# leospeidel/Colate

Hardware: AMD Instinct MI355X
Metric: bootstrap replicates/sec to EM convergence, whole-genome SGDP mut, 20 epochs (higher is better)
Workload: dtype f64

## Files before the change

### colate_amd/csrc/em_kernel_impl.hpp

```cpp
#pragma once
#include <hip/hip_runtime.h>

#include <cstdlib>
#include <cstring>
#include <type_traits>

#include "em_kernels.h"
#include "em_math.hpp"

namespace {

constexpr int kWave = 64;
enum { O_W = 0, O_N, O_D, kNumBinArrays };
enum { G_LAM = 0, G_INV, G_XA, G_P, G_BETA, G_CS, G_S, G_PW, kNumGather };
constexpr int G_Q = kNumGather;
constexpr int num_gather_rows(int nch, bool tput) { return (nch >= 2 || !tput) ? kNumGather + 1 : kNumGather; }
constexpr int tail_scratch_arrays(int nch, bool tput) { return nch >= 2 ? (tput ? 3 : 6) : 0; }

__device__ __forceinline__ double readlane_d(double v, int lane) {
  int lo = __builtin_amdgcn_readlane(__double2loint(v), lane);
  int hi = __builtin_amdgcn_readlane(__double2hiint(v), lane);
  return __hiloint2double(hi, lo);
}

template <int CTRL, int ROW_MASK = 0xf, bool BOUND = false>
__device__ __forceinline__ double dpp_d(double old, double v) {
  int lo = __builtin_amdgcn_update_dpp(__double2loint(old), __double2loint(v), CTRL, ROW_MASK, 0xf, BOUND);
  int hi = __builtin_amdgcn_update_dpp(__double2hiint(old), __double2hiint(v), CTRL, ROW_MASK, 0xf, BOUND);
  return __hiloint2double(hi, lo);
}
constexpr int ROW_SHR1 = 0x111, ROW_SHR2 = 0x112, ROW_SHR4 = 0x114, ROW_SHR8 = 0x118;
constexpr int ROW_SHL1 = 0x101, ROW_SHL2 = 0x102, ROW_SHL4 = 0x104, ROW_SHL8 = 0x108;
constexpr int ROW_BCAST15 = 0x142, ROW_BCAST31 = 0x143, WAVE_SHR1 = 0x138, WAVE_SHL1 = 0x130;


__device__ __forceinline__ double wave_prefix_sum(double v, int rows = 4) {
  v += dpp_d<ROW_SHR1, 0xf, true>(0.0, v);
  v += dpp_d<ROW_SHR2, 0xf, true>(0.0, v);
  v += dpp_d<ROW_SHR4, 0xf, true>(0.0, v);
  v += dpp_d<ROW_SHR8, 0xf, true>(0.0, v);
  if (rows > 1) v += dpp_d<ROW_BCAST15, 0xa>(0.0, v);
  if (rows > 2) v += dpp_d<ROW_BCAST31, 0xc>(0.0, v);
  return v;
}
__device__ __forceinline__ double wave_suffix_sum(double v, int lane, int rows = 4) {
  v += dpp_d<ROW_SHL1, 0xf, true>(0.0, v);
  v += dpp_d<ROW_SHL2, 0xf, true>(0.0, v);
  v += dpp_d<ROW_SHL4, 0xf, true>(0.0, v);
  v += dpp_d<ROW_SHL8, 0xf, true>(0.0, v);
  if (rows > 1) {
    const double r1 = readlane_d(v, 16);
    double add = 0.0;
    if (rows > 2) {
      const double r2 = readlane_d(v, 32), r3 = readlane_d(v, 48);
      const double s23 = r2 + r3, s123 = r1 + s23;
      const int row = lane >> 4;
      add = row == 0 ? s123 : (row == 1 ? s23 : (row == 2 ? r3 : 0.0));
    } else {
      add = (lane >> 4) == 0 ? r1 : 0.0;
    }
    v = v + add;
  }
  return v;
}
__device__ __forceinline__ void wave_affine_scan(double& a, double& b, int rows = 4, const double* nosrc = nullptr) {
#define COLATE_AFF_STEP(CTRL, RM, BND, K)                                                                   \
  {                                                                                                         \
    const double as = nosrc ? dpp_d<CTRL, RM, true>(0.0, a) + nosrc[K] : dpp_d<CTRL, RM>(1.0, a);           \
    const double bs = dpp_d<CTRL, RM, BND>(0.0, b);                                                         \
    b = em::fma_(a, bs, b);                                                                                 \
    a = a * as;                                                                                             \
  }
  COLATE_AFF_STEP(ROW_SHR1, 0xf, true, 0)
  COLATE_AFF_STEP(ROW_SHR2, 0xf, true, 1)
  COLATE_AFF_STEP(ROW_SHR4, 0xf, true, 2)
  COLATE_AFF_STEP(ROW_SHR8, 0xf, true, 3)
#undef COLATE_AFF_STEP
  if (rows == 2) {
    const double bs = dpp_d<ROW_BCAST15, 0xa>(0.0, b);
    b = em::fma_(a, bs, b);
  }
#define COLATE_AFF_STEP2(CTRL, RM)                 \
  {                                                \
    const double as = dpp_d<CTRL, RM>(1.0, a);     \
    const double bs = dpp_d<CTRL, RM>(0.0, b);     \
    b = em::fma_(a, bs, b);                        \
    a = a * as;                                    \
  }
  if (rows > 2) COLATE_AFF_STEP2(ROW_BCAST15, 0xa)
  if (rows > 2) COLATE_AFF_STEP2(ROW_BCAST31, 0xc)
#undef COLATE_AFF_STEP2
}

__device__ __forceinline__ double wave_suffix_max(double v, int lane) {
  v = __builtin_fmax(v, dpp_d<ROW_SHL1, 0xf, true>(0.0, v));
  v = __builtin_fmax(v, dpp_d<ROW_SHL2, 0xf, true>(0.0, v));
  v = __builtin_fmax(v, dpp_d<ROW_SHL4, 0xf, true>(0.0, v));
  v = __builtin_fmax(v, dpp_d<ROW_SHL8, 0xf, true>(0.0, v));
  const double r1 = readlane_d(v, 16), r2 = readlane_d(v, 32), r3 = readlane_d(v, 48);
  const double m23 = __builtin_fmax(r2, r3), m123 = __builtin_fmax(r1, m23);
  const int row = lane >> 4;
  return __builtin_fmax(v, row == 0 ? m123 : (row == 1 ? m23 : (row == 2 ? r3 : 0.0)));
}
__device__ __forceinline__ double half_ulp_pos(double z) {
  const int ex = (__double2hiint(z) >> 20) & 0x7ff;
  return ex > 53 ? __hiloint2double((ex - 53) << 20, 0) : 0.0;
}

__device__ __forceinline__ double tail_hneg(double z, double& q) {
  const float a = __builtin_fminf(__builtin_fabsf((float)z), 30.0f);
  const float t = __builtin_amdgcn_rcpf(__builtin_fmaf(0.2316419f, a, 1.0f));
  float poly = __builtin_fmaf(t, 1.330274429f, -1.821255978f);
  poly = __builtin_fmaf(t, poly, 1.781477937f);
  poly = __builtin_fmaf(t, poly, -0.356563782f);
  poly = __builtin_fmaf(t, poly, 0.319381530f);
  poly = poly * t;
  const float phi = 0.3989422804f * __builtin_amdgcn_exp2f(-0.72134752f * (a * a));
  const float qa = phi * poly;
  const float base = __builtin_fmaxf(__builtin_fmaf(-a, qa, phi), 0.0f);
  q = z < 0.0 ? (double)(1.0f - qa) : (double)qa;
  return (z < 0.0 ? -z : 0.0) + (double)base;
}

#ifdef COLATE_EM_STAMPS
__device__ __forceinline__ unsigned long long stamp() {
  unsigned long long t;
  __builtin_amdgcn_sched_barrier(0);
  asm volatile("s_memtime %0\n\ts_waitcnt lgkmcnt(0)" : "=s"(t)::"memory");
  __builtin_amdgcn_sched_barrier(0);
  return t;
}
#define COLATE_STAMP(i)                     \
  {                                         \
    const unsigned long long now_ = stamp(); \
    st_acc[i] += now_ - st_prev;            \
    st_prev = now_;                         \
  }
#define COLATE_PSTAMP(i) pro_t[i] = stamp();
#else
#define COLATE_STAMP(i)
#define COLATE_PSTAMP(i)
#endif

#ifdef COLATE_ABL
#define COLATE_ABL_HAS(b) (((COLATE_ABL) >> (b)) & 1)
#else
#define COLATE_ABL_HAS(b) 0
#endif

#define COLATE_COLD() asm volatile("; cold path")
#define COLATE_STR2(x) #x
#define COLATE_STR(x) COLATE_STR2(x)

__device__ __forceinline__ bool finite_pos(double x) { return x > 0.0 && x < __builtin_inf(); }

__device__ __forceinline__ unsigned long long ballot64(bool p) { return __builtin_amdgcn_ballot_w64(p); }

__device__ __forceinline__ void wave_lds_fence() {
  __builtin_amdgcn_fence(__ATOMIC_RELEASE, "wavefront");
  __builtin_amdgcn_wave_barrier();
  __builtin_amdgcn_fence(__ATOMIC_ACQUIRE, "wavefront");
}

struct BinStat {
  double a_b, cnt, tk, tkn, dtk, da, db;
  double f1, f2, f4, f8;
  int kb, pos;
  bool live, last_bin, is_tail;
};
enum { BF_F1 = 1, BF_F2 = 2, BF_F4 = 4, BF_F8 = 8, BF_TAIL = 16, BF_INRANGE = 32, BF_KB_SHIFT = 8 };

constexpr int em_loop_pad(int mode, int nch, int erows, bool tput, int wpe) {
#ifdef COLATE_LOOP_PAD
  return (COLATE_LOOP_PAD) & 7;
#else
  (void)erows, (void)wpe;
  if (mode != 0) return 0;
#ifdef COLATE_EM_ILP_BUILD
  (void)tput;
  return nch == 1 ? (wpe == 2 ? 5 : 6) : 2;
#else
  (void)nch;
  if (!tput) return 6;
  return 4;
#endif
#endif
}

constexpr int em_loop_pad2(int mode, int nch, bool tput) {
#if defined(COLATE_EM_ILP_BUILD) && !defined(COLATE_LOOP_PAD)
  (void)mode, (void)nch, (void)tput;
  return -1;
#else
  (void)mode, (void)nch, (void)tput;
  return -1;
#endif
}

template <int MODE, int NCH, int EROWS, bool TPUT, int WPE = 0>
__global__ __launch_bounds__(TPUT ? 2 * kWave : 2 * COLATE_EM_MAX_A, WPE ? WPE : ((NCH == 1) ? 3 : (NCH == 2 ? 2 : 1))) void em_kernel(ColateEmArgs p) {
  extern __shared__ double lds[];
  const int E = p.E, A = p.A;
  constexpr int EPAD = NCH * kWave;
  const int NBMAX = (A + kWave - 1) / kWave;
  const int AP = NBMAX * kWave;
  const int APZ = AP + 2;
  const int tid = threadIdx.x, lane = tid & 63;
  constexpr int kSlotShift = (NCH == 1) ? 0 : (NCH == 2 ? 1 : (NCH == 4 ? 2 : (NCH == 8 ? 3 : 4)));
  static_assert(NCH == 1 || NCH == 2 || NCH == 4 || NCH == 8 || NCH == 16, "NCH");
  auto ep_of = [&](int c) { return lane * NCH + c; };
  const int wave = __builtin_amdgcn_readfirstlane(tid >> 6);
  const int role = wave & 1;
  const int grp = wave >> 1;
  const int rep = blockIdx.x;

  double* s_t = lds;
  double* s_ep = s_t + EPAD + 1;
  constexpr int kRows = num_gather_rows(NCH, TPUT);
  double* s_out = s_ep + kRows * EPAD;
  double* s_nd = s_out + 2 * kNumBinArrays * APZ;
  double* s_cfail = s_nd + 4 * EPAD;
  double* s_cnt = s_cfail + 2 * APZ;
  double* s_ll = s_cnt + 2 * APZ;
  double* s_exptab = s_ll + 12;
  double* s_age = s_exptab + em::kExpTableDoubles;
  double* s_tscr = s_age + AP;
  int* s_kb = reinterpret_cast<int*>(s_tscr + tail_scratch_arrays(NCH, TPUT) * APZ);
  int* s_fail = s_kb + AP + 1;
  int* s_misc = s_fail + 8;
  int* s_bflags = s_misc + 4;

#ifdef COLATE_EM_TRACE
  unsigned long long trace_t0;
  asm volatile("s_memtime %0\n\ts_waitcnt lgkmcnt(0)" : "=s"(trace_t0)::"memory");
#endif
#ifdef COLATE_EM_STAMPS
  unsigned long long pro_t[10] = {0, 0, 0, 0, 0, 0, 0, 0, 0, 0};
#endif
  COLATE_PSTAMP(0)
  const double* epochs = p.epochs + (size_t)rep * p.epochs_stride;
  for (int i = tid; i < EPAD + 1; i += blockDim.x) s_t[i] = (i < E) ? epochs[i] : 0.0;
  for (int i = tid; i < kRows * EPAD + 2 * kNumBinArrays * APZ + 4 * EPAD + 4 * APZ; i += blockDim.x) s_ep[i] = 0.0;
  if (tid == 0) {
    s_misc[0] = A;
    s_misc[1] = 0;
    s_misc[2] = 0;
    s_misc[3] = 0;
  }
  if (tid < 8) {
    s_ll[tid] = 0.0;
    s_fail[tid] = 0;
  }
  if (tid < em::kExpTableDoubles) s_exptab[tid] = em::kExpTableDevice[tid];
  __syncthreads();
  COLATE_PSTAMP(1)
  for (int t = tid; t < AP; t += blockDim.x) {
    int kb = E;
    bool has_sh = false, has_ns = false;
    if (t < A) {
      const double a = p.age_grid[t];
      const double c1 = p.cnt_sh[(size_t)rep * A + t];
      const double c2 = p.cnt_ns[(size_t)rep * A + t];
      const double csh = (c1 > 0) ? c1 : 0.0;
      const double cns = (c2 > 0) ? c2 : 0.0;
      int first_gt = 0;
      for (int len = E; len > 0;) {
        const int half = len >> 1;
        if (!(a < s_t[first_gt + half])) {
          first_gt += half + 1;
          len -= half + 1;
        } else {
          len = half;
        }
      }
      kb = first_gt - 1;
      if (kb < 0) kb = 0;
      s_cnt[t] = csh;
      s_cnt[APZ + t] = cns;
      s_age[t] = a;
      has_sh = csh > 0;
      has_ns = cns > 0;
    }
    {
      const unsigned long long m_sh = ballot64(has_sh), m_ns = ballot64(has_ns), m_any = m_sh | m_ns;
      if (m_any != 0 && lane == 0) {
        atomicMin(&s_misc[0], t + (int)__builtin_ctzll(m_any));
        atomicMax(&s_misc[1], t + 64 - (int)__builtin_clzll(m_any));
        atomicAdd(&s_misc[3], (int)__builtin_popcountll(m_sh) + (int)__builtin_popcountll(m_ns));
      }
    }
    s_kb[t] = kb;
  }
  if (tid == 0) s_kb[AP] = E + 1;
  __syncthreads();
  COLATE_PSTAMP(2)
  int nzlo = s_misc[0], nzhi = s_misc[1];
  if (nzlo >= nzhi) {
    nzlo = 0;
    nzhi = 0;
  }
  const int NB = (nzhi - nzlo + 63) / 64 > 0 ? (nzhi - nzlo + 63) / 64 : 1;

  double t_e[NCH], tn_e[NCH], dt_e[NCH], lam_e[NCH];
  bool vstat[NCH], ep_on[NCH];
#pragma unroll
  for (int c = 0; c < NCH; c++) {
    const int e = ep_of(c);
    ep_on[c] = e < E;
    t_e[c] = s_t[e];
    tn_e[c] = 0.0;
    dt_e[c] = 0.0;
    vstat[c] = false;
    lam_e[c] = 0.0;
    if (ep_on[c]) {
      if (e < E - 1) {
        tn_e[c] = s_t[e + 1];
        dt_e[c] = tn_e[c] - t_e[c];
        vstat[c] = (tn_e[c] != 0) && (dt_e[c] > 0);
      } else {
        vstat[c] = true;
      }
      lam_e[c] = p.rates_in[(size_t)rep * p.rates_stride + e];
      if (MODE == 0 && wave == 0) p.out_rates[(size_t)rep * E + e] = lam_e[c];
    }
  }
  COLATE_PSTAMP(3)
  if (tid == 0) s_ll[10] = (nzhi > nzlo) ? (double)s_kb[nzhi - 1] : -1.0;
  const int pos = grp * kWave + lane;
  const int bin = nzlo + pos;
  const bool in_range = (grp < NB) && (bin < nzhi);
  double a_b = 0, cnt = 0, tk = 0, tkn = 0, dtk = 0, da = 0, db = 0;
  int kb = E;
  if (in_range) {
    a_b = p.age_grid[bin];
    cnt = s_cnt[role * APZ + bin];
    kb = s_kb[bin];
    tk = s_t[kb];
    if (kb < E - 1) {
      tkn = s_t[kb + 1];
      dtk = tkn - tk;
    }
    da = a_b - tk;
    db = (kb < E - 1) ? tkn - a_b : 0.0;
  }
  const bool live = in_range && cnt > 0;
  const bool last_bin = (kb == E - 1);
  double f1 = 0, f2 = 0, f4 = 0, f8 = 0;
  bool is_tail = false;
  if (in_range) {
    const int r = lane & 15;
    if (r >= 1 && s_kb[bin - 1] == kb) f1 = 1.0;
    if (r >= 2 && s_kb[bin - 2] == kb) f2 = 1.0;
    if (r >= 4 && s_kb[bin - 4] == kb) f4 = 1.0;
    if (r >= 8 && s_kb[bin - 8] == kb) f8 = 1.0;
    is_tail = (r == 15) || (bin + 1 >= nzhi) || (s_kb[bin + 1] != kb);
  }
  const BinStat bs0{a_b, cnt, tk, tkn, dtk, da, db, f1, f2, f4, f8, kb, pos, live, last_bin, is_tail};
  if (TPUT) {
    for (int t = tid; t < AP; t += blockDim.x) {
      const int b = nzlo + t;
      int fl = 0;
      if (t < NB * kWave && b < nzhi) {
        const int k = s_kb[b], r = t & 15;
        fl = BF_INRANGE | (k << BF_KB_SHIFT);
        if (r >= 1 && s_kb[b - 1] == k) fl |= BF_F1;
        if (r >= 2 && s_kb[b - 2] == k) fl |= BF_F2;
        if (r >= 4 && s_kb[b - 4] == k) fl |= BF_F4;
        if (r >= 8 && s_kb[b - 8] == k) fl |= BF_F8;
        if (r == 15 || b + 1 >= nzhi || s_kb[b + 1] != k) fl |= BF_TAIL;
      }
      s_bflags[t] = fl;
    }
  }
  int slot0[NCH], slot1[NCH], slot2[NCH], row_x[NCH], row_hi[NCH], seg_hi[NCH];
  int nlt[NCH];
  double C0[NCH];
  constexpr double kIntegResidue = 4.0e-17;
  constexpr double kResolvedRatio = 1.0e10;
  COLATE_PSTAMP(4)
  double c_all = 0.0;
  for (int b = nzlo; b < nzhi; b += 8) {
    double v[8];
#pragma unroll
    for (int j = 0; j < 8; j++) v[j] = s_cnt[role * APZ + b + j];
#pragma unroll
    for (int j = 0; j < 8; j++) c_all += (b + j < nzhi) ? v[j] : 0.0;
  }
  COLATE_PSTAMP(5)
#ifdef COLATE_TAIL_CONST_HOLD
  constexpr bool kLinearHold = false;
#else
  constexpr bool kLinearHold = (NCH >= 2);
#endif
  double eta_e[NCH], eta_s[NCH];
#pragma unroll
  for (int c = 0; c < NCH; c++) eta_e[c] = 0.0, eta_s[c] = 1.0;
  bool tail_trivial_prev = true;
  if (tid < 2 * kWave && lane == 0) s_ll[8 + role] = c_all;
#pragma unroll
  for (int c = 0; c < NCH; c++) {
    const int e = ep_of(c);
    int lo = A, hi = 0, n_before = 0;
    double c_later = 0.0;
    if (ep_on[c]) {
      lo = hi = 0;
      for (int len = A; len > 0;) {
        const int half = len >> 1;
        if (s_kb[lo + half] < e) {
          lo += half + 1;
          len -= half + 1;
        } else {
          len = half;
        }
      }
      for (int len = A; len > 0;) {
        const int half = len >> 1;
        if (s_kb[hi + half] <= e) {
          hi += half + 1;
          len -= half + 1;
        } else {
          len = half;
        }
      }
      const int lo_c = lo < nzlo ? nzlo : (lo > nzhi ? nzhi : lo);
      n_before = lo_c - nzlo;
    }
    {
      int b0 = __builtin_amdgcn_readfirstlane(hi);
      if (b0 < nzlo) b0 = nzlo;
      for (int b = b0; b < nzhi; b += 8) {
        double v[8];
#pragma unroll
        for (int j = 0; j < 8; j++) v[j] = s_cnt[role * APZ + b + j];
#pragma unroll
        for (int j = 0; j < 8; j++) {
          c_later += (ep_on[c] && b + j >= hi && b + j < nzhi) ? v[j] : 0.0;
        }
      }
    }
    C0[c] = c_later;
    nlt[c] = n_before;
    const int clo = (lo > nzlo ? lo : nzlo) - nzlo, chi = (hi < nzhi ? hi : nzhi) - nzlo;
    seg_hi[c] = chi;
    slot0[c] = slot1[c] = slot2[c] = AP;
    row_x[c] = 1;
    row_hi[c] = 0;
    if (clo < chi) {
      const int r0 = clo >> 4, r1 = (chi - 1) >> 4;
      slot0[c] = (r0 * 16 + 15 < chi - 1) ? r0 * 16 + 15 : chi - 1;
      if (r1 > r0) slot1[c] = ((r0 + 1) * 16 + 15 < chi - 1) ? (r0 + 1) * 16 + 15 : chi - 1;
      if (r1 > r0 + 1) slot2[c] = ((r0 + 2) * 16 + 15 < chi - 1) ? (r0 + 2) * 16 + 15 : chi - 1;
      row_x[c] = r0 + 3;
      row_hi[c] = r1;
    }
  }
  if (role == 0) {
    const double from_below = dpp_d<WAVE_SHR1, 0xf, true>(0.0, C0[NCH - 1]);
#pragma unroll
    for (int c = 0; c < NCH; c++) {
      const double c_ge = (c == 0) ? (lane == 0 ? c_all : from_below) : C0[c - 1];
      eta_e[c] = dt_e[c] * (kIntegResidue * c_ge);
    }
  }
  bool more_rows[NCH];
  bool third_row = false;
#pragma unroll
  for (int c = 0; c < NCH; c++) {
    more_rows[c] = (ballot64(row_x[c] <= row_hi[c]) != 0);
    third_row |= (ballot64(slot2[c] != AP) != 0);
  }
  __syncthreads();
  COLATE_PSTAMP(6)
  if (!TPUT && grp >= NB) return;
  const bool leader = (grp == 0);
  constexpr bool kFreeBuild = !TPUT && NCH == 1 && WPE == 2;
  const int verdict_wave = (!TPUT && NB >= 2 && NCH != 2) ? (kFreeBuild ? 1 : 2) : 0;
  const bool tracker = (wave == verdict_wave);
  constexpr int erows = EROWS;
  constexpr bool kFree = kFreeBuild;
  double aff_nosrc[4] = {0.0, 0.0, 0.0, 0.0};
  if (kFree) {
    aff_nosrc[0] = (lane & 15) < 1 ? 1.0 : 0.0;
    aff_nosrc[1] = (lane & 15) < 2 ? 1.0 : 0.0;
    aff_nosrc[2] = (lane & 15) < 4 ? 1.0 : 0.0;
    aff_nosrc[3] = (lane & 15) < 8 ? 1.0 : 0.0;
  }
  const int p1b_wave = (kFree && NB >= 2) ? 3 : 1;
  const int nwave_live = 2 * NB;
  (void)nwave_live;

  int my_flags = 0;
  constexpr double kTinyNum = 1e-280;
  unsigned tr_min[NCH], tr_max[NCH];
  int tr_noisy = 0;
#pragma unroll
  for (int c = 0; c < NCH; c++) tr_min[c] = 0xffffffffu, tr_max[c] = 0u;
  constexpr double kNoisyRatio = 1.0e6;
  double noisy_thr[NCH];
#pragma unroll
  for (int c = 0; c < NCH; c++)
    noisy_thr[c] = (double)(ep_of(c)) <= s_ll[10] ? kNoisyRatio * (dt_e[c] * (kIntegResidue * (s_ll[8] + s_ll[9]))) : 0.0;
  unsigned long long prev_fail = 0;
  unsigned long long ep_mask[NCH];
#pragma unroll
  for (int c = 0; c < NCH; c++) ep_mask[c] = ballot64(ep_on[c]);
  const double thr = 1.0 - p.rel_tol;
  double ll = -__builtin_inf(), prev_ll = -__builtin_inf();
  int iter = 0;
  const int max_iter = (MODE == 1) ? 1 : p.max_iter;
  double* out_mine = s_out + role * kNumBinArrays * APZ;

#ifdef COLATE_EM_STAMPS
  unsigned long long st_acc[16] = {0, 0, 0, 0, 0, 0, 0, 0, 0, 0, 0, 0, 0, 0, 0, 0};
  COLATE_PSTAMP(7)
  unsigned long long st_prev = stamp();
#endif
  constexpr int kPad = em_loop_pad(MODE, NCH, EROWS, TPUT, WPE);
#define COLATE_PAD_CASE(n) \
  if constexpr (kPad == n) asm volatile(".p2align 6\n\t.rept " #n "\n\ts_nop 0\n\t.endr");
#define COLATE_LOOP_ANCHOR()                                            \
  {                                                                     \
    COLATE_PAD_CASE(0) COLATE_PAD_CASE(1) COLATE_PAD_CASE(2) COLATE_PAD_CASE(3) \
    COLATE_PAD_CASE(4) COLATE_PAD_CASE(5) COLATE_PAD_CASE(6) COLATE_PAD_CASE(7) \
  }
  bool last_pos = true;
  int lim = 0;
  constexpr bool kAssumeAbsorbing = kFree || TPUT;
  unsigned long long last_bit[NCH];
#pragma unroll
  for (int c = 0; c < NCH; c++) last_bit[c] = (((E - 1) & (NCH - 1)) == c) ? 1ull << (((E - 1) >> kSlotShift) & 63) : 0ull;
  auto last_rate_positive = [&]() {
    unsigned long long pos = 0;
#pragma unroll
    for (int c = 0; c < NCH; c++) pos |= ballot64(lam_e[c] > 0.0) & last_bit[c];
    return pos != 0ull;
  };
  const unsigned long long last_bit1 = 1ull << ((E - 1) & 63);
  if (kFree) last_pos = (ballot64(lam_e[0] > 0.0) & last_bit1) != 0ull;
  if (TPUT) last_pos = last_rate_positive();
  auto tail_due = [&](int it) {
#ifdef COLATE_TAIL_LATE256
    if (NCH >= 2) return it < 128 ? (it & (it - 1)) == 0 : (it < 512 ? (it & 127) == 0 : (it & 255) == 0);
#else
    if (NCH >= 2) return it < 128 ? (it & (it - 1)) == 0 : (it & 127) == 0;
#endif
    return (it & (it - 1)) == 0 || (!tail_trivial_prev && (it & 31) == 0);
  };
  auto tail_next_due = [&](int it) {
    if (it <= 1) return it;
    const int p2 = 1 << (32 - __builtin_clz((unsigned)(it - 1)));
#ifdef COLATE_TAIL_LATE256
    if (NCH >= 2) return it <= 128 ? p2 : (it <= 512 ? ((it + 127) & ~127) : ((it + 255) & ~255));
#else
    if (NCH >= 2) return it <= 128 ? p2 : ((it + 127) & ~127);
#endif
    const int m32 = (it + 31) & ~31;
    return (!tail_trivial_prev && m32 < p2) ? m32 : p2;
  };
  auto iteration = [&](auto role_c, auto leader_c, auto ll_c, auto track_c, auto refresh_c, auto p1_c) __attribute__((always_inline)) -> bool {
    COLATE_STAMP(7)
    constexpr int kRole = decltype(role_c)::value, kLeader = decltype(leader_c)::value, kNeedLL = decltype(ll_c)::value;
    constexpr int kTrack = decltype(track_c)::value;
    constexpr int kRefresh = decltype(refresh_c)::value;
    constexpr bool kSteady = (kNeedLL >= 0);
    const int ROLE = kRole < 0 ? role : kRole;
    const bool LEADER = kLeader < 0 ? leader : (kLeader != 0);
    constexpr bool kSplit = (kLeader >= 2);
    constexpr int kOwn = (kLeader == 3) ? 1 : 0;
    static_assert(!kSplit || NCH == 2, "the split is for two epochs per lane");
    auto own = [&](int c) { return !kSplit || c == kOwn; };
    constexpr int kP1 = decltype(p1_c)::value;
    const bool P1A = kP1 < 0 ? (ROLE == 0 && (kFree || LEADER)) : ((kP1 & 1) != 0);
    const bool P1B = kP1 < 0 ? (kFree ? wave == p1b_wave : (LEADER && ROLE == 1)) : ((kP1 & 2) != 0);
    constexpr bool CROSS = kFree;
    const bool need_ll = kNeedLL < 0 ? ((MODE == 1) || (iter >= p.min_iter) || (iter == max_iter - 1) || p.ll_trace != nullptr) : (kNeedLL != 0);
    double q_e[NCH], p_e[NCH], beta_e[NCH], S_e[NCH], omS_e[NCH], cs_e[NCH];
#pragma unroll
    for (int c = 0; c < NCH; c++) q_e[c] = p_e[c] = beta_e[c] = S_e[c] = omS_e[c] = cs_e[c] = 0.0;
    if ((P1A || P1B) && !COLATE_ABL_HAS(15)) {
      double x_e[NCH];
#pragma unroll
      for (int c = 0; c < NCH; c++) x_e[c] = lam_e[c] * dt_e[c];
      if (P1A) {
        double loc[NCH];
        loc[0] = 0.0;
#pragma unroll
        for (int c = 1; c < NCH; c++) loc[c] = loc[c - 1] + x_e[c - 1];
        const double tot = (NCH == 1) ? x_e[0] : loc[NCH - 1] + x_e[NCH - 1];
#if COLATE_ABL_HAS(11)
        const double incl = tot * 7.0;
#else
        const double incl = wave_prefix_sum(tot, erows);
#endif
        const double excl = dpp_d<WAVE_SHR1, 0xf, true>(0.0, incl);
#pragma unroll
        for (int c = 0; c < NCH; c++) cs_e[c] = (c == 0) ? excl : excl + loc[c];
      }
      COLATE_STAMP(8)
      if (P1A) {
#pragma unroll
        for (int c = 0; c < NCH; c++) {
          if (!own(c)) continue;
          const int e = ep_of(c);
#if COLATE_ABL_HAS(3)
          S_e[c] = 1.0 - cs_e[c] * 1e-3;
          omS_e[c] = cs_e[c] * 1e-3;
#else
          S_e[c] = em::em_exp_om_t<true>(cs_e[c], &omS_e[c], s_exptab);
#endif
          if (!kFree || LEADER) {
            s_ep[G_CS * EPAD + e] = cs_e[c];
            s_ep[G_S * EPAD + e] = S_e[c];
            s_ep[G_PW * EPAD + e] = omS_e[c];
          }
        }
      }
      if (P1B) {
#pragma unroll
        for (int c = 0; c < NCH; c++) {
          if (!own(c)) continue;
          const int e = ep_of(c);
#if COLATE_ABL_HAS(7)
          const double inv = 2.0e4 - lam_e[c];
#else
          const double inv = em::em_rcp_ieee(lam_e[c]);
#endif
          const bool valid = vstat[c] && (lam_e[c] > 0);
#if COLATE_ABL_HAS(4)
          const double qx = 1.0 - x_e[c];
#else
          const double qx = em::em_exp_t(-x_e[c], s_exptab);
#endif
          q_e[c] = (e < E - 1) ? qx : 0.0;
          p_e[c] = valid ? 1.0 - q_e[c] : 0.0;
          beta_e[c] = valid ? (t_e[c] + inv) - (tn_e[c] + inv) * q_e[c] : 0.0;
          s_ep[G_LAM * EPAD + e] = lam_e[c];
          if (!CROSS) {
            s_ep[G_INV * EPAD + e] = inv;
#if COLATE_ABL_HAS(7)
            s_ep[G_XA * EPAD + e] = (t_e[c] + inv) * lam_e[c];
#else
            s_ep[G_XA * EPAD + e] = em::em_div_known_rcp(t_e[c] + inv, inv, lam_e[c]);
#endif
          }
          s_ep[G_P * EPAD + e] = p_e[c];
          s_ep[G_BETA * EPAD + e] = beta_e[c];
          if (NCH >= 2 || kFree) s_ep[G_Q * EPAD + e] = q_e[c];
        }
      }
    }
    double lk_pre = 0.0;
    if (!TPUT) {
      const int kq = bs0.kb < E ? bs0.kb : 0;
#pragma unroll
      for (int c = 0; c < NCH; c++) {
        const int lo = __builtin_amdgcn_ds_bpermute(((kq >> kSlotShift) & 63) << 2, __double2loint(lam_e[c]));
        const int hi = __builtin_amdgcn_ds_bpermute(((kq >> kSlotShift) & 63) << 2, __double2hiint(lam_e[c]));
        if (NCH == 1 || (kq & (NCH - 1)) == c) lk_pre = __hiloint2double(hi, lo);
      }
      asm volatile("" : "+v"(lk_pre));
    }
    double Sk_pre = 0.0, PWk_pre = 0.0, qd_pre = 0.0;
    if (kFree && ROLE == 0) {
      const int kq = bs0.kb < E ? bs0.kb : 0;
      const int s_lo = __builtin_amdgcn_ds_bpermute((kq & 63) << 2, __double2loint(S_e[0]));
      const int s_hi = __builtin_amdgcn_ds_bpermute((kq & 63) << 2, __double2hiint(S_e[0]));
      const int o_lo = __builtin_amdgcn_ds_bpermute((kq & 63) << 2, __double2loint(omS_e[0]));
      const int o_hi = __builtin_amdgcn_ds_bpermute((kq & 63) << 2, __double2hiint(omS_e[0]));
      Sk_pre = __hiloint2double(s_hi, s_lo);
      PWk_pre = __hiloint2double(o_hi, o_lo);
      qd_pre = em::em_exp_t(-(lk_pre * bs0.da), s_exptab);
    }
    COLATE_STAMP(9)
    bool absorbing = kAssumeAbsorbing && kSteady;
    if (!(kAssumeAbsorbing && kSteady)) {
      const int cl = (E - 1) & (NCH - 1), ll_ = (E - 1) >> kSlotShift;
#pragma unroll
      for (int c = 0; c < NCH; c++) {
        const unsigned long long pos = ballot64(lam_e[c] > 0.0);
        if (NCH == 1 || c == cl) absorbing = (pos >> ll_) & 1ull;
      }
    }
    if (!kFree || need_ll || !absorbing) __syncthreads();
    COLATE_STAMP(0)
    auto bin_terms = [&](const BinStat& bs, const double lk_own, const bool have_lk, const bool cross, const double Sk_in, const double PWk_in, const double qd_in) {
      const double a_b = bs.a_b, cnt = bs.cnt, tk = bs.tk, tkn = bs.tkn, dtk = bs.dtk, da = bs.da, db = bs.db;
      const double f1 = bs.f1, f2 = bs.f2, f4 = bs.f4, f8 = bs.f8;
      const int kb = bs.kb, pos = bs.pos;
      const bool live = bs.live, last_bin = bs.last_bin, is_tail = bs.is_tail;
      const int wslot = 2 * (pos >> 6) + ROLE;
      double o_w = 0, o_N = 0, o_D = 0, llp = 0.0;
      bool fail = false;
      unsigned long long fail_direct = 0;
      bool have_fail_direct = false;
      if (ROLE == 0 && !COLATE_ABL_HAS(12)) {
        const double lk = have_lk ? lk_own : s_ep[G_LAM * EPAD + kb];
        const bool lpos = lk > 0;
        const double ik = cross ? (lpos ? em::em_rcp_ieee(lk) : 0.0) : s_ep[G_INV * EPAD + kb];
        const double Sk = cross ? Sk_in : s_ep[G_S * EPAD + kb], PWk = cross ? PWk_in : s_ep[G_PW * EPAD + kb];
        const double Xak = cross ? em::em_div_known_rcp(tk + ik, ik, lk) : s_ep[G_XA * EPAD + kb];
#if COLATE_ABL_HAS(5)
        const double qd = 1.0 - lk * da;
#else
        const double qd = cross ? qd_in : em::em_exp_t(-(lk * da), s_exptab);
#endif
#if COLATE_ABL_HAS(8)
        const double Y = (a_b + ik) * lk;
#else
        const double Y = em::em_div_known_rcp(a_b + ik, ik, lk);
#endif
        const double Wp = (cross || lpos) ? Sk * (1.0 - qd) : 0.0;
        const double X = Xak - Y * qd;
        const double Vp = (cross || lpos) ? X * ik * Sk : 0.0;
        const double Sig = PWk + Wp;
        const bool fin = finite_pos(Sig), ok = live && fin;
        const double r = ok ? em::em_rcp(Sig) : 0.0;
        const double nk = Wp * r;
        double dk = Vp * r + (-tk * nk);
        dk = __builtin_fmax(dk, 0.0);
        o_w = cnt * r;
        o_N = cnt * nk;
        o_D = cnt * dk;
        fail_direct = ballot64(live) & ~ballot64(fin);
        have_fail_direct = true;
        if (need_ll) {
          COLATE_COLD();
          llp = ok ? cnt * em::em_log(Sig) : 0.0;
        }
      } else if (ROLE == 1 && !COLATE_ABL_HAS(12)) {
        const double lk = have_lk ? lk_own : s_ep[G_LAM * EPAD + kb];
        const double ik = cross ? em::em_rcp_ieee(lk) : s_ep[G_INV * EPAD + kb];
        const bool lpos = lk > 0;
        auto neg_cs_age = [&]() {
          const double ck = s_ep[G_CS * EPAD + kb];
          const double ck1 = ck + lk * da;
          return -(ck1 + lk * (a_b - a_b));
        };
#if COLATE_ABL_HAS(6)
        const double u = 1.0 - lk * db;
#else
        const double u = em::em_exp_t(-(lk * db), s_exptab);
#endif
        const double pn = 1.0 - u;
        const double bn = lpos ? (a_b + ik) - (tkn + ik) * u : 0.0;
        {
          double dk = bn + (-tk * pn + dtk * (1.0 - pn));
          dk = __builtin_fmax(dk, 0.0);
          o_w = cnt * u;
          o_N = cnt * pn;
          o_D = cnt * dk;
          if (need_ll) {
            COLATE_COLD();
            llp = live ? cnt * neg_cs_age() : 0.0;
          }
        }
        if (__builtin_expect(!absorbing, 0)) {
          COLATE_COLD();
          o_w = o_N = o_D = llp = 0.0;
          if (live) {
            const double Gk1 = 1.0 - em::em_exp_t(-s_ep[G_CS * EPAD + E - 1] + s_ep[G_CS * EPAD + kb + 1], s_exptab);
            const double SigN = pn + u * Gk1;
            if (finite_pos(SigN)) {
              const double rr = 1.0 / SigN;
              const double nk = pn * rr;
              double dk = bn * rr + (-tk * nk + dtk * (1.0 - nk));
              dk = __builtin_fmax(dk, 0.0);
              o_w = cnt * (u * rr);
              o_N = cnt * nk;
              o_D = cnt * dk;
              llp = cnt * (neg_cs_age() + em::em_log(SigN));
            } else {
              fail = true;
            }
          }
        }
        if (__builtin_expect(ballot64(last_bin && live) != 0, 0)) {
          COLATE_COLD();
          if (last_bin && live) {
            if (!lpos) my_flags |= COLATE_FLAG_NAN;
            double dk = (a_b + ik) - tk;
            dk = __builtin_fmax(dk, 0.0);
            o_w = 0.0;
            o_N = cnt;
            o_D = cnt * dk;
            fail = false;
            llp = need_ll ? cnt * neg_cs_age() : 0.0;
          }
        }
      }
      COLATE_STAMP(1)
      unsigned char* s_failb = reinterpret_cast<unsigned char*>(s_fail);
      const unsigned long long fail_mask = have_fail_direct ? fail_direct : ballot64(fail);
      if (have_fail_direct) fail = (fail_mask >> lane) & 1ull;
      if (TPUT) {
        s_cfail[ROLE * APZ + pos] = fail ? cnt : 0.0;
        if (lane == 0) s_failb[ROLE * 4 + (pos >> 6)] = fail_mask ? 1 : 0;
      } else {
        const unsigned long long touch = fail_mask | prev_fail;
        if (__builtin_expect(touch != 0, 0)) {
          COLATE_COLD();
          if ((touch >> lane) & 1ull) s_cfail[ROLE * APZ + pos] = fail ? cnt : 0.0;
          if ((fail_mask != 0) != (prev_fail != 0)) {
            if (lane == 0) s_failb[ROLE * 4 + (pos >> 6)] = fail_mask ? 1 : 0;
          }
          prev_fail = fail_mask;
        }
      }
#define COLATE_SEG_STEP(CTRL, F)                              \
  o_w = em::fma_(dpp_d<CTRL, 0xf, true>(0.0, o_w), F, o_w);   \
  o_N = em::fma_(dpp_d<CTRL, 0xf, true>(0.0, o_N), F, o_N);   \
  o_D = em::fma_(dpp_d<CTRL, 0xf, true>(0.0, o_D), F, o_D);
#if !COLATE_ABL_HAS(2)
      COLATE_SEG_STEP(ROW_SHR1, f1)
      COLATE_SEG_STEP(ROW_SHR2, f2)
      COLATE_SEG_STEP(ROW_SHR4, f4)
      COLATE_SEG_STEP(ROW_SHR8, f8)
#endif
#undef COLATE_SEG_STEP
      {
        const int tpos = is_tail ? pos : AP + 1;
        out_mine[O_W * APZ + tpos] = o_w;
        out_mine[O_N * APZ + tpos] = o_N;
        out_mine[O_D * APZ + tpos] = o_D;
      }
      if (need_ll) {
        COLATE_COLD();
        const double tot = readlane_d(wave_prefix_sum(llp), 63);
        if (lane == 0) s_ll[wslot] = tot;
      }
    };
    if (TPUT) {
      for (int g = 0; g < NB; g++) {
        const int gpos = g * kWave + lane, fl = s_bflags[gpos], gbin = nzlo + gpos;
        const bool inr = fl & BF_INRANGE;
        BinStat b;
        b.kb = inr ? (fl >> BF_KB_SHIFT) : 0;
        b.pos = gpos;
        b.a_b = inr ? s_age[gbin] : 0.0;
        b.cnt = inr ? s_cnt[ROLE * APZ + gbin] : 0.0;
        b.tk = s_t[b.kb];
        b.tkn = (b.kb < E - 1) ? s_t[b.kb + 1] : 0.0;
        b.dtk = (b.kb < E - 1) ? b.tkn - b.tk : 0.0;
        b.da = b.a_b - b.tk;
        b.db = (b.kb < E - 1) ? b.tkn - b.a_b : 0.0;
        b.f1 = (fl & BF_F1) ? 1.0 : 0.0;
        b.f2 = (fl & BF_F2) ? 1.0 : 0.0;
        b.f4 = (fl & BF_F4) ? 1.0 : 0.0;
        b.f8 = (fl & BF_F8) ? 1.0 : 0.0;
        b.live = inr && b.cnt > 0;
        b.last_bin = (b.kb == E - 1);
        b.is_tail = fl & BF_TAIL;
        bin_terms(b, 0.0, false, false, 0.0, 0.0, 0.0);
      }
    } else {
      bin_terms(bs0, lk_pre, true, CROSS, Sk_pre, PWk_pre, qd_pre);
    }
    COLATE_STAMP(2)
    __syncthreads();
    if constexpr (em_loop_pad2(MODE, NCH, TPUT) >= 0) {
      static_assert(em_loop_pad2(MODE, NCH, TPUT) < 0 || em_loop_pad2(MODE, NCH, TPUT) == 4, "add the asm for another pad");
      asm volatile(".p2align 5\n\t.rept 4\n\ts_nop 0\n\t.endr");
    }
    COLATE_STAMP(3)
    if (LEADER && !COLATE_ABL_HAS(13)) {
      const int anyf = s_fail[ROLE];
      double w[NCH], oN[NCH], oD[NCH];
#pragma unroll
      for (int c = 0; c < NCH; c++) w[c] = oN[c] = oD[c] = 0.0;
#pragma unroll
      for (int c = 0; c < NCH; c++) {
        const bool mine = own(c);
#if COLATE_ABL_HAS(1)
        const double w0 = 1e-3 * lane, w1 = 0, w2 = 0, n0 = 1e-3, n1 = 0, n2 = 0, d0 = 1.0, d1 = 0, d2 = 0;
#else
        const double w0 = out_mine[O_W * APZ + slot0[c]], w1 = out_mine[O_W * APZ + slot1[c]];
        const double w2 = kSteady ? 0.0 : out_mine[O_W * APZ + slot2[c]];
        double n0 = 0, n1 = 0, n2 = 0, d0 = 0, d1 = 0, d2 = 0;
        if (mine) {
          n0 = out_mine[O_N * APZ + slot0[c]], n1 = out_mine[O_N * APZ + slot1[c]];
          d0 = out_mine[O_D * APZ + slot0[c]], d1 = out_mine[O_D * APZ + slot1[c]];
          n2 = kSteady ? 0.0 : out_mine[O_N * APZ + slot2[c]];
          d2 = kSteady ? 0.0 : out_mine[O_D * APZ + slot2[c]];
        }
#endif
        if (ROLE == 0 && mine) {
          p_e[c] = s_ep[G_P * EPAD + ep_of(c)];
          beta_e[c] = s_ep[G_BETA * EPAD + ep_of(c)];
        }
        if (ROLE == 1 && mine && !P1B) {
          q_e[c] = s_ep[G_Q * EPAD + ep_of(c)];
          p_e[c] = s_ep[G_P * EPAD + ep_of(c)];
          beta_e[c] = s_ep[G_BETA * EPAD + ep_of(c)];
        }
        w[c] = kSteady ? (w0 + w1) : (w0 + w1) + w2;
        oN[c] = kSteady ? (n0 + n1) : (n0 + n1) + n2;
        oD[c] = (kSteady ? (d0 + d1) : (d0 + d1) + d2);
        if (ROLE == 0) oD[c] = oD[c] + eta_e[c];
        if (!kSteady && __builtin_expect(more_rows[c], 0)) for (int r = row_x[c]; r <= row_hi[c]; r++) {
          COLATE_COLD();
          int slot = r * 16 + 15;
          if (slot > seg_hi[c] - 1) slot = seg_hi[c] - 1;
          w[c] += out_mine[O_W * APZ + slot];
          oN[c] += out_mine[O_N * APZ + slot];
          oD[c] += out_mine[O_D * APZ + slot];
        }
      }
      COLATE_STAMP(10)
      double Cn[NCH];
#pragma unroll
      for (int c = 0; c < NCH; c++) Cn[c] = C0[c];
      {
        if (__builtin_expect(anyf != 0, 0)) {
          COLATE_COLD();
#pragma unroll
          for (int c = 0; c < NCH; c++) {
            double fs = 0.0;
            for (int q = seg_hi[c] > 0 ? seg_hi[c] : 0; ep_on[c] && q < nzhi - nzlo; q++) {
              if (s_kb[nzlo + q] > ep_of(c)) fs += s_cfail[ROLE * APZ + q];
            }
            Cn[c] -= fs;
          }
        }
      }
      double Npart[NCH], Dpart[NCH];
      if (ROLE == 0) {
        double RSn[NCH], ls[NCH];
        ls[NCH - 1] = 0.0;
#pragma unroll
        for (int c = NCH - 2; c >= 0; c--) ls[c] = ls[c + 1] + w[c + 1];
        {
          const double tot = (NCH == 1) ? w[0] : ls[0] + w[0];
#if COLATE_ABL_HAS(9)
          const double sR = tot * 3.0;
#else
          const double sR = wave_suffix_sum(tot, lane, erows);
#endif
          const double excl = dpp_d<WAVE_SHL1, 0xf, true>(0.0, sR);
#pragma unroll
          for (int c = 0; c < NCH; c++) RSn[c] = (c == NCH - 1) ? excl : excl + ls[c];
        }
        COLATE_STAMP(11)
#pragma unroll
        for (int c = 0; c < NCH; c++) {
          Npart[c] = Dpart[c] = 0.0;
          if (!own(c)) continue;
          const int e = ep_of(c);
          const double W = S_e[c] * p_e[c];
          const double VW = S_e[c] * beta_e[c] - t_e[c] * W;
          const double PWn = omS_e[c] + W;
          Npart[c] = W * RSn[c] + oN[c];
          double integ = Cn[c] - PWn * RSn[c];
          integ = __builtin_fmax(integ, 0.0);
          double dsh = VW * RSn[c] + dt_e[c] * integ;
          dsh = __builtin_fmax(dsh, 0.0);
          Dpart[c] = dsh + oD[c];
          (void)e;
        }
      } else {
        double T[NCH];
        {
          double qa[NCH], wb[NCH];
#pragma unroll
          for (int c = 0; c < NCH; c++) {
            if (kSplit && !own(c)) q_e[c] = s_ep[G_Q * EPAD + ep_of(c)];
            qa[c] = ep_on[c] ? q_e[c] : 1.0;
            wb[c] = ep_on[c] ? w[c] : 0.0;
          }
          double a = qa[0], b = wb[0];
#pragma unroll
          for (int c = 1; c < NCH; c++) {
            b = em::fma_(qa[c], b, wb[c]);
            a = a * qa[c];
          }
#if !COLATE_ABL_HAS(9)
          wave_affine_scan(a, b, erows, kFree ? aff_nosrc : nullptr);
#endif
          T[0] = dpp_d<WAVE_SHR1, 0xf, true>(0.0, b);
#pragma unroll
          for (int c = 1; c < NCH; c++) T[c] = em::fma_(qa[c - 1], T[c - 1], wb[c - 1]);
        }
        COLATE_STAMP(12)
        if constexpr (kRefresh != 0) {
          const bool due = kRefresh > 0 || tail_due(iter);
          if (__builtin_expect(due, kRefresh > 0)) {
            if (kRefresh < 0) COLATE_COLD();
            const int k_old = (int)s_ll[10];
            const int e_o1 = (k_old + 1 < E - 1) ? (k_old + 1 > 0 ? k_old + 1 : 0) : E - 1;
            const double S_old1 = s_ep[G_S * EPAD + e_o1];
            double S1[NCH], We[NCH];
            bool alive_l[NCH], dead_l[NCH];
            unsigned long long between[NCH], small_w[NCH], any_between = 0;
#pragma unroll
            for (int c = 0; c < NCH; c++) {
              const int e = ep_of(c);
              const bool has = e < E - 1;
              const double pe = (kSplit && !own(c)) ? s_ep[G_P * EPAD + e] : p_e[c];
              We[c] = ep_on[c] ? s_ep[G_S * EPAD + e] * pe : 0.0;
              S1[c] = has ? s_ep[G_S * EPAD + e + 1] : 1.0;
              const double Ie = (NCH == 1) ? q_e[c] * T[c] : S1[c] * (c_all - C0[c]);
              alive_l[c] = !has || nlt[c] == 0 ||
                           ((e > k_old) ? S1[c] >= 1e-11 : (S1[c] >= 1e-14 && Ie >= 1e-8 * (c_all - C0[c])));
              dead_l[c] = has && e > k_old && S1[c] < 4e-20 * S_old1;
              between[c] = ballot64(ep_on[c] && !(alive_l[c] || dead_l[c]));
              any_between |= between[c];
              small_w[c] = ballot64(ep_on[c] && We[c] < 0x1p-53 * 0.37 && We[c] > 0.0);
            }
            const bool trivial = (any_between == 0);
            if (!(trivial && tail_trivial_prev && (iter & 255) != 0)) {
              tail_trivial_prev = trivial;
              int e_sm = E;
#pragma unroll
              for (int c = 0; c < NCH; c++)
                if (small_w[c]) {
                  const int e1 = __builtin_ctzll(small_w[c]) * NCH + c;
                  e_sm = e1 < e_sm ? e1 : e_sm;
                }
              double* const scr = s_tscr + (kSplit ? kOwn * 3 * APZ : 0);
              double* const s_w = (NCH == 1) ? out_mine + O_W * APZ : scr;
              double* const s_a = (NCH == 1) ? out_mine + O_N * APZ : scr + APZ;
              double* const s_d = (NCH == 1) ? out_mine + O_D * APZ : scr + 2 * APZ;
              double PDtot = 0.0, PHtot = 0.0, PMtot = 0.0;
              for (int g = 0; g < NB; g++) {
                const int gpos = g * kWave + lane, gbin = nzlo + gpos;
                const bool inr = gbin < nzhi;
                const int kbb = inr ? s_kb[inr ? gbin : 0] : E;
                const double cntb = inr ? s_cnt[APZ + (inr ? gbin : 0)] : 0.0;
                const bool liveb = inr && cntb > 0 && kbb < E - 1;
                const int kq = liveb ? kbb : 0;
                const double ab = liveb ? s_age[gbin] : 0.0, tkb = s_t[kq], tknb = s_t[kq + 1];
                const double lkb = s_ep[G_LAM * EPAD + kq], ckb = s_ep[G_CS * EPAD + kq];
                const double csa = ckb + lkb * (ab - tkb);
                const double th = half_ulp_pos(csa);
                const double mb = em::em_exp_t(__builtin_fmin(csa, 230.0), s_exptab);
                double Db = 0.0;
                int ndrop = 0;
                for (int eb = e_sm & ~(NCH - 1); eb < E; eb += NCH) {
#pragma unroll
                  for (int c = 0; c < NCH; c++) {
                    const int e = eb + c;
                    const double w = readlane_d(We[c], eb >> kSlotShift) * mb;
                    const bool dr = (e < E) && (e > kq) && (w < th);
                    Db += dr ? w : 0.0;
                    ndrop += dr ? 1 : 0;
                  }
                }
                const int nfold = E - 1 - kq - ndrop;
                const double xk = lkb * (tknb - tkb);
                double nh = (double)(E - kq);
                if (xk > 0.0) nh = __builtin_fmin(0.69 * em::em_rcp(xk), nh);
                nh += 1.5;
                const double sb = __builtin_amdgcn_sqrt((0x1p-108 / 3.0) * nh + th * th * ((double)nfold * (1.0 / 3.0)));
                const double rsb = em::em_rcp(sb);
                const double wv = liveb ? cntb * sb : 0.0, av = liveb ? mb * rsb : 0.0, dv = liveb ? Db * rsb : 0.0;
                s_w[gpos] = wv;
                s_a[gpos] = av;
                s_d[gpos] = dv;
                double qd;
                const double ch = wv * tail_hneg(dv, qd);
                const double cm = liveb ? cntb * mb : 0.0, cd = liveb ? cntb * Db : 0.0;
                PHtot = PHtot + readlane_d(wave_prefix_sum(ch), 63);
                PMtot = PMtot + readlane_d(wave_prefix_sum(cm), 63);
                PDtot = PDtot + readlane_d(wave_prefix_sum(cd), 63);
              }
              wave_lds_fence();
#pragma unroll
              for (int c = 0; c < NCH; c++) {
                const int e = ep_of(c);
                double Ra = alive_l[c] ? ((e > k_old) ? -PDtot : 0.0) : PHtot;
                double Rb = alive_l[c] ? 0.0 : -PMtot;
                for (unsigned long long m = own(c) ? between[c] : 0ull; m != 0; m &= m - 1) {
                  const int l = __builtin_ctzll(m);
                  const double S1e = readlane_d(S1[c], l);
                  const int nlte = __builtin_amdgcn_readlane(nlt[c], l);
                  double acc = 0.0, acc1 = 0.0;
                  for (int g = 0; g < NB; g++) {
                    const int gpos = g * kWave + lane;
                    const double dv = s_d[gpos], av = s_a[gpos], wv = s_w[gpos];
                    double qz;
                    const double term = wv * (tail_hneg(S1e * av - dv, qz) - dv);
                    acc += (gpos < nlte) ? term : 0.0;
                    acc1 += (gpos < nlte) ? (wv * av) * qz : 0.0;
                  }
                  const double r0 = readlane_d(wave_prefix_sum(acc), 63), r1 = -readlane_d(wave_prefix_sum(acc1), 63);
                  Ra = (lane == l) ? r0 - r1 * S1e : Ra;
                  Rb = (lane == l) ? r1 : Rb;
                }
                const bool on = ep_on[c] && e < E - 1;
                if (kLinearHold) {
                  const double X0 = q_e[c] * T[c];
                  const bool lin = on && own(c) && X0 > 0.0;
                  eta_e[c] = on ? (lin ? Ra : Ra + Rb * S1[c]) : 0.0;
                  eta_s[c] = lin ? 1.0 + Rb * (S1[c] * em::em_rcp(X0)) : 1.0;
                } else {
                  eta_e[c] = on ? Ra + Rb * S1[c] : 0.0;
                }
              }
            }
          }
        }
#pragma unroll
        for (int c = 0; c < NCH; c++) {
          Npart[c] = Dpart[c] = 0.0;
          if (!own(c)) continue;
          const int e = ep_of(c);
          Npart[c] = p_e[c] * T[c] + oN[c];
          double Gn = kLinearHold ? eta_s[c] : 1.0;
          if (__builtin_expect(!absorbing, 0)) {
            COLATE_COLD();
            if (e < E - 1) Gn = (1.0 - em::em_exp_t(-s_ep[G_CS * EPAD + E - 1] + s_ep[G_CS * EPAD + e + 1], s_exptab)) + (Gn - 1.0);
          }
          const double integ_ns = __builtin_fmax(Gn * (q_e[c] * T[c]) + eta_e[c], 0.0);
          double dns = dt_e[c] * Cn[c] + ((beta_e[c] - t_e[c] * p_e[c]) * T[c] + dt_e[c] * integ_ns);
          dns = __builtin_fmax(dns, 0.0);
          Dpart[c] = dns + oD[c];
        }
      }
#pragma unroll
      for (int c = 0; c < NCH; c++) {
        if (!own(c)) continue;
        s_nd[(ROLE * 2 + 0) * EPAD + ep_of(c)] = Npart[c];
        s_nd[(ROLE * 2 + 1) * EPAD + ep_of(c)] = Dpart[c];
      }
    }
    COLATE_STAMP(4)
    __syncthreads();
    COLATE_STAMP(6)
    double N_e[NCH], D_e[NCH];
#pragma unroll
    for (int c = 0; c < NCH; c++) {
      const int e = ep_of(c);
      N_e[c] = s_nd[0 * EPAD + e] + s_nd[2 * EPAD + e];
      D_e[c] = s_nd[1 * EPAD + e] + s_nd[3 * EPAD + e];
      if (MODE == 1 && ep_on[c]) {
        if (N_e[c] != N_e[c] || D_e[c] != D_e[c]) my_flags |= COLATE_FLAG_NAN;
        if (N_e[c] < 0.0 || D_e[c] < 0.0) my_flags |= COLATE_FLAG_NEG;
      }
    }
    COLATE_STAMP(13)
    if (need_ll) {
      COLATE_COLD();
      ll = ((s_ll[0] + s_ll[1]) + (s_ll[2] + s_ll[3])) + ((s_ll[4] + s_ll[5]) + (s_ll[6] + s_ll[7]));
      if (kNeedLL < 0 && p.ll_trace && tid == 0 && iter < p.ll_trace_cap) p.ll_trace[(size_t)rep * p.ll_trace_cap + iter] = ll;
    }
    if (MODE == 1) {
      if (wave == 0) {
#pragma unroll
        for (int c = 0; c < NCH; c++) {
          if (ep_on[c]) {
            p.out_num[(size_t)rep * E + ep_of(c)] = N_e[c];
            p.out_den[(size_t)rep * E + ep_of(c)] = D_e[c];
          }
        }
      }
      return true;
    }
    if (!COLATE_ABL_HAS(14)) {
      double cand[NCH];
      bool self[NCH];
      unsigned long long keep[NCH];
      unsigned long long cpm[NCH];
#pragma unroll
      for (int c = 0; c < NCH; c++) {
        const bool copy = (N_e[c] == 0);
        {
#if COLATE_ABL_HAS(10)
          double qn = N_e[c] * 1e-4 + D_e[c] * 1e-9;
#else
          double qn = N_e[c] / D_e[c];
#endif
          qn = em::max_c(qn, p.rate_floor);
          cand[c] = (!copy && D_e[c] != 0) ? qn : lam_e[c];
        }
        const unsigned long long zero_n = __builtin_amdgcn_fcmp(N_e[c], 0.0, 1 );
        keep[c] = ep_mask[c] & ~zero_n;
        cpm[c] = ep_mask[c] & zero_n;
        self[c] = ep_on[c] && !copy;
      }
      unsigned long long bad = (NCH == 1) ? 0ull : (cpm[0] & ~((cpm[NCH - 1] << 1) | 1ull));
#pragma unroll
      for (int c = 0; c < NCH; c++) {
        bad |= cpm[c] & (cpm[c] + 1ull);
        if (c > 0) bad |= cpm[c] & ~cpm[c - 1];
      }
      if (kTrack < 0 ? tracker : (kTrack != 0)) {
#pragma unroll
        for (int c = 0; c < NCH; c++) {
          const unsigned nh = (unsigned)__double2hiint(N_e[c]);
          tr_min[c] = nh < tr_min[c] ? nh : tr_min[c];
          tr_max[c] = nh > tr_max[c] ? nh : tr_max[c];
          tr_noisy |= (ep_on[c] && N_e[c] != 0.0 && D_e[c] < noisy_thr[c] && cand[c] > p.rate_floor) ? 1 : 0;
        }
      }
      if (__builtin_expect(bad == 0, 1)) {
#pragma unroll
        for (int c = 0; c < NCH; c++) lam_e[c] = self[c] ? cand[c] : 0.0;
      } else {
        COLATE_COLD();
        unsigned long long any_keep = 0;
        double lastc = 0.0;
#pragma unroll
        for (int c = 0; c < NCH; c++) {
          any_keep |= keep[c];
          lastc = self[c] ? cand[c] : lastc;
        }
        const unsigned long long below = any_keep & ((1ull << lane) - 1ull);
        const int src = below ? 63 - __builtin_clzll(below) : 0;
        const double from_lanes = __shfl(lastc, src, 64);
        double prev = below ? from_lanes : 0.0;
#pragma unroll
        for (int c = 0; c < NCH; c++) {
          lam_e[c] = ep_on[c] ? (self[c] ? cand[c] : prev) : 0.0;
          prev = self[c] ? cand[c] : prev;
        }
      }
    }
    if (kAssumeAbsorbing && kSteady) {
      lim = (kFree ? ((ballot64(lam_e[0] > 0.0) & last_bit1) != 0ull) : last_rate_positive()) ? lim : 0;
      asm volatile("" : "+s"(lim));
    }
    COLATE_STAMP(5)
    bool stop = false;
    if (kNeedLL != 0 && iter > p.min_iter) {
      COLATE_COLD();
      stop = (ll / prev_ll > thr);
    }
    prev_ll = ll;
    return stop;
  };
  bool stopped = false;
  if constexpr (NCH <= 4) if (MODE == 0 && p.ll_trace == nullptr) {
    int n_steady = p.min_iter < max_iter - 1 ? p.min_iter : max_iter - 1;
    if (n_steady < 0) n_steady = 0;
    using C0 = std::integral_constant<int, 0>;
    using C1 = std::integral_constant<int, 1>;
    using CR = std::integral_constant<int, -1>;
#define COLATE_STEADY(R, L, T, P)                             \
  {                                                           \
    lim = n_steady;                                           \
    COLATE_LOOP_ANCHOR()                                      \
    do {                                                      \
      iteration(R{}, L{}, C0{}, T{}, C0{}, P{});              \
    } while (__builtin_expect(++iter < lim, 1));              \
    if (kAssumeAbsorbing && lim == 0) last_pos = false;                  \
  }
#define COLATE_STEADY_B(R, L, T, P)                                                    \
  while (iter < n_steady && last_pos) {                                                \
    if (tail_due(iter)) {                                                              \
      lim = n_steady;                                                                  \
      iteration(R{}, L{}, C0{}, T{}, C1{}, P{});                                       \
      ++iter;                                                                          \
      if (kAssumeAbsorbing && lim == 0) last_pos = false;                                         \
      if (iter >= n_steady || !last_pos) break;                                        \
    }                                                                                  \
    lim = tail_next_due(iter);                                                         \
    if (lim > n_steady) lim = n_steady;                                                \
    COLATE_LOOP_ANCHOR()                                                               \
    while (__builtin_expect(iter < lim, 1)) {                                          \
      iteration(R{}, L{}, C0{}, T{}, C0{}, P{});                                       \
      ++iter;                                                                          \
    }                                                                                  \
    if (kAssumeAbsorbing && lim == 0) last_pos = false;                                           \
  }
    bool any_more_rows = false;
#pragma unroll
    for (int c = 0; c < NCH; c++) any_more_rows |= more_rows[c];
#define COLATE_STEADY_LL(R, L, T, P)                          \
  if (last_pos) {                                             \
    lim = max_iter;                                           \
    COLATE_LOOP_ANCHOR()                                      \
    for (; iter < lim; iter++) {                              \
      if (iteration(R{}, L{}, C1{}, T{}, C0{}, P{})) {        \
        stopped = true;                                       \
        break;                                                \
      }                                                       \
    }                                                         \
    if (kAssumeAbsorbing && lim == 0) last_pos = false;                  \
  }
#define COLATE_STEADY_LL_B(R, L, T, P)                                                 \
// ... 254 lines not shown
```

Measured before the change: 110,000.

## Hoist multiplicative half of wave affine scan out of the critical path

Splits the wave-level affine prefix scan into a rate part (products of q) and a data part (fma on b). For the steady, non-throughput, single-channel, two-waves-per-EU role-1 leader variant, the rate part is computed early, right after the q values are produced, and only the data part runs in the dependent section. This shortens the serial DPP chain on the hot path. In exchange it recomputes q via exp instead of reading it from LDS and keeps six extra doubles live in registers. It also lowers the loop pad for that configuration from 5 to 2.

```diff
diff --git a/colate_amd/csrc/em_kernel_impl.hpp b/colate_amd/csrc/em_kernel_impl.hpp
--- a/colate_amd/csrc/em_kernel_impl.hpp
+++ b/colate_amd/csrc/em_kernel_impl.hpp
@@ -91,6 +91,30 @@
   if (rows > 2) COLATE_AFF_STEP2(ROW_BCAST31, 0xc)
 #undef COLATE_AFF_STEP2
 }
+constexpr int kAffSteps = 6;
+__device__ __forceinline__ void wave_affine_scan_rates(double a, double (&am)[kAffSteps], int rows, const double* nosrc) {
+  am[0] = a;
+#define COLATE_AFF_STEP(CTRL, RM, K)                                                                        \
+  {                                                                                                         \
+    const double as = nosrc ? dpp_d<CTRL, RM, true>(0.0, a) + nosrc[K] : dpp_d<CTRL, RM>(1.0, a);           \
+    a = a * as;                                                                                             \
+    am[K + 1] = a;                                                                                          \
+  }
+  COLATE_AFF_STEP(ROW_SHR1, 0xf, 0)
+  COLATE_AFF_STEP(ROW_SHR2, 0xf, 1)
+  COLATE_AFF_STEP(ROW_SHR4, 0xf, 2)
+  COLATE_AFF_STEP(ROW_SHR8, 0xf, 3)
+#undef COLATE_AFF_STEP
+  am[5] = rows > 2 ? a * dpp_d<ROW_BCAST15, 0xa>(1.0, a) : a;
+}
+__device__ __forceinline__ void wave_affine_scan_data(const double (&am)[kAffSteps], double& b, int rows) {
+  b = em::fma_(am[0], dpp_d<ROW_SHR1, 0xf, true>(0.0, b), b);
+  b = em::fma_(am[1], dpp_d<ROW_SHR2, 0xf, true>(0.0, b), b);
+  b = em::fma_(am[2], dpp_d<ROW_SHR4, 0xf, true>(0.0, b), b);
+  b = em::fma_(am[3], dpp_d<ROW_SHR8, 0xf, true>(0.0, b), b);
+  if (rows > 1) b = em::fma_(am[4], dpp_d<ROW_BCAST15, 0xa>(0.0, b), b);
+  if (rows > 2) b = em::fma_(am[5], dpp_d<ROW_BCAST31, 0xc>(0.0, b), b);
+}
 
 __device__ __forceinline__ double wave_suffix_max(double v, int lane) {
   v = __builtin_fmax(v, dpp_d<ROW_SHL1, 0xf, true>(0.0, v));
@@ -178,7 +202,7 @@
   if (mode != 0) return 0;
 #ifdef COLATE_EM_ILP_BUILD
   (void)tput;
-  return nch == 1 ? (wpe == 2 ? 5 : 6) : 2;
+  return nch == 1 ? (wpe == 2 ? 2 : 6) : 2;
 #else
   (void)nch;
   if (!tput) return 6;
@@ -194,6 +218,15 @@
 #else
   (void)mode, (void)nch, (void)tput;
   return -1;
+#endif
+}
+
+constexpr bool em_affine_split(int nch, bool tput, int wpe) {
+#ifdef COLATE_AFFINE_SPLIT
+  (void)nch, (void)tput, (void)wpe;
+  return (COLATE_AFFINE_SPLIT) != 0;
+#else
+  return !tput && nch == 1 && wpe == 2;
 #endif
 }
 
@@ -648,6 +681,23 @@
           if (NCH >= 2 || kFree) s_ep[G_Q * EPAD + e] = q_e[c];
         }
       }
+    }
+    constexpr bool kHoist = em_affine_split(NCH, TPUT, WPE) && kSteady && kNeedLL == 0 && kRole == 1 && kLeader == 1;
+    double aff_m[kAffSteps];
+    if constexpr (kHoist) {
+      double a = 1.0;
+#pragma unroll
+      for (int c = 0; c < NCH; c++) {
+        if (!P1B) {
+          const double qx = em::em_exp_t(-(lam_e[c] * dt_e[c]), s_exptab);
+          q_e[c] = (ep_of(c) < E - 1) ? qx : 0.0;
+        }
+        const double qa = ep_on[c] ? q_e[c] : 1.0;
+        a = (c == 0) ? qa : a * qa;
+      }
+      wave_affine_scan_rates(a, aff_m, erows, kFree ? aff_nosrc : nullptr);
+#pragma unroll
+      for (int k = 0; k < (erows > 2 ? 6 : (erows > 1 ? 5 : 4)); k++) asm volatile("" : "+v"(aff_m[k]));
     }
     double lk_pre = 0.0;
     if (!TPUT) {
@@ -888,7 +938,7 @@
           beta_e[c] = s_ep[G_BETA * EPAD + ep_of(c)];
         }
         if (ROLE == 1 && mine && !P1B) {
-          q_e[c] = s_ep[G_Q * EPAD + ep_of(c)];
+          if (!kHoist) q_e[c] = s_ep[G_Q * EPAD + ep_of(c)];
           p_e[c] = s_ep[G_P * EPAD + ep_of(c)];
           beta_e[c] = s_ep[G_BETA * EPAD + ep_of(c)];
         }
@@ -973,7 +1023,11 @@
             a = a * qa[c];
           }
 #if !COLATE_ABL_HAS(9)
-          wave_affine_scan(a, b, erows, kFree ? aff_nosrc : nullptr);
+          if constexpr (kHoist) {
+            wave_affine_scan_data(aff_m, b, erows);
+          } else {
+            wave_affine_scan(a, b, erows, kFree ? aff_nosrc : nullptr);
+          }
 #endif
           T[0] = dpp_d<WAVE_SHR1, 0xf, true>(0.0, b);
 #pragma unroll
```

Measured after the change: 112,000, median of 6. +1.8%, better.
